# mingfeisun/DeepMimic_mujoco

Hardware: AMD Instinct MI355X
Metric: env-steps/sec (higher is better)
Workload: dtype f64

## Files before the change

### deepmimic_mujoco_amd/csrc/slot_step.h

```cpp
#pragma once

#include "env_step.h"
#include "slot_kernel.h"

namespace dm {

template <class R> struct DofVec { R r[DOF_PASSES]; };

template <class R>
DM_DEV void slot_integrate_pos(SlotShared<R>& s, const DofVec<R>& x0q, int sl, R h) {
  const R q0 = dmw::row_bcast<3>(x0q.r[0]), q1 = dmw::row_bcast<4>(x0q.r[0]), q2 = dmw::row_bcast<5>(x0q.r[0]), q3 = dmw::row_bcast<6>(x0q.r[0]);
  if (sl < 3) s.qpos[sl] = x0q.r[0] + h * s.tau[sl];
  else if (sl == 3) {
    R ax[3] = {s.tau[3], s.tau[4], s.tau[5]}, q[4] = {q0, q1, q2, q3}, qr[4];
    const R angle = h * normalize3(ax);
    if (angle == R(0)) { qr[0] = 1; qr[1] = qr[2] = qr[3] = 0; } else axisangle2quat(qr, ax, angle);
    normalize4(q);
    quat_mul(q, q, qr);
    s.qpos[3] = q[0]; s.qpos[4] = q[1]; s.qpos[5] = q[2]; s.qpos[6] = q[3];
  } else if (sl >= 7) s.qpos[sl] = x0q.r[0] + h * s.tau[sl - 1];
#pragma unroll
  for (int c = 1; c < Q_PASSES; c++) { const int i = sl + SW * c; if (i < NQ) s.qpos[i] = x0q.r[c] + h * s.tau[i - 1]; }
}

template <class R, bool PROF = false, bool CARRY = false, int MAXR = 2 * SW>
DM_DEV void slot_rk4_step(const DevModel<R>& M, SlotShared<R>& s, const SlotTables& tb, int sl, int lane, const LaneTopo& lt, R* xip, int& ovf, long long* prof = 0) {
  const R h = M.timestep;
  const R A[3] = {R(0.5), R(0.5), R(1)};
  const R Bw[4] = {R(1) / 6, R(1) / 3, R(1) / 3, R(1) / 6};
  DofVec<R> x0q, x0v, vprev, aprev, sumv, suma;
#pragma unroll
  for (int c = 0; c < DOF_PASSES; c++) {
    const int i = sl + SW * c;
    x0q.r[c] = i < NQ ? s.qpos[i] : R(0);
    const R v0 = i < NV ? s.qvel[i] : R(0);
    x0v.r[c] = v0; vprev.r[c] = v0; aprev.r[c] = 0; sumv.r[c] = 0; suma.r[c] = 0;
  }
  dmw::sync();
  for (int i = 0; i < 4; i++) {
    if (i > 0) {
      const R cf = A[i - 1];
#pragma unroll
      for (int c = 0; c < DOF_PASSES; c++) { const int d = sl + SW * c; if (d < NV) s.tau[d] = cf * vprev.r[c]; }
      dmw::sync();
      slot_integrate_pos(s, x0q, sl, h);
#pragma unroll
      for (int c = 0; c < DOF_PASSES; c++) {
        const int d = sl + SW * c;
        if (d < NV) { const R vi = x0v.r[c] + h * (cf * aprev.r[c]); vprev.r[c] = vi; s.qvel[d] = vi; }
      }
      dmw::sync();
    }
    typedef decltype(dmw::park(R(0))) ParkedR;
    ParkedR pk[5][DOF_PASSES];
#pragma unroll
    for (int c = 0; c < DOF_PASSES; c++) { pk[0][c] = dmw::park(x0q.r[c]); pk[1][c] = dmw::park(x0v.r[c]); pk[2][c] = dmw::park(vprev.r[c]); pk[3][c] = dmw::park(sumv.r[c]); pk[4][c] = dmw::park(suma.r[c]); }
    slot_forward<R, PROF, CARRY, MAXR>(M, s, tb, sl, lane, lt, xip, ovf, (const DebugOut*)0, prof);
#pragma unroll
    for (int c = 0; c < DOF_PASSES; c++) { x0q.r[c] = dmw::unpark(pk[0][c]); x0v.r[c] = dmw::unpark(pk[1][c]); vprev.r[c] = dmw::unpark(pk[2][c]); sumv.r[c] = dmw::unpark(pk[3][c]); suma.r[c] = dmw::unpark(pk[4][c]); }
#pragma unroll
    for (int c = 0; c < DOF_PASSES; c++) {
      const int d = sl + SW * c;
      if (d < NV) { const R a = s.qd.o.qacc[d]; aprev.r[c] = a; sumv.r[c] += Bw[i] * vprev.r[c]; suma.r[c] += Bw[i] * a; }
    }
  }
#pragma unroll
  for (int c = 0; c < DOF_PASSES; c++) { const int d = sl + SW * c; if (d < NV) s.tau[d] = sumv.r[c]; }
  dmw::sync();
  slot_integrate_pos(s, x0q, sl, h);
#pragma unroll
  for (int c = 0; c < DOF_PASSES; c++) { const int d = sl + SW * c; if (d < NV) { s.qvel[d] = x0v.r[c] + h * suma.r[c]; s.qws[d] = aprev.r[c]; } }
  dmw::sync();
}

template <class R>
DM_DEV void slot_load_env(const DevModel<R>& M, const Batch<R>& B, SlotShared<R>& s, int env, int sl, bool live, const double* action, int n_substeps = 1) {
#pragma unroll
  for (int c = 0; c < Q_PASSES; c++) {
    const int i = sl + SW * c;
    if (i < NQ) s.qpos[i] = B.qpos[(size_t)env * NQ + i];
    if (i < NV) { s.qvel[i] = B.qvel[(size_t)env * NV + i]; s.qws[i] = B.qws[(size_t)env * NV + i]; s.act[i] = 0; }
  }
  if (sl == 0) { s.status = 0; s.nefc = 0; s.ncon = 0; s.solver_iter = 0; }
  dmw::sync();
  if (action) {
#pragma unroll
    for (int c = 0; c < HINGE_PASSES; c++) {
      const int u = sl + SW * c;
      if (u < NU) {
        const R a = ctrl_of_action(M, B, env, u, (R)action[(size_t)env * NU + u], s.qpos[7 + u], s.qvel[6 + u], n_substeps);
        if (live) B.ctrl[(size_t)env * NU + u] = a;
        s.act[u + 6] = act_force(M, u + 6, a);
      }
    }
  }
  dmw::sync_mem();
}

template <class R, bool CARRY = false>
DM_DEV void slot_spd_control(const DevModel<R>& M, const Batch<R>& B, SlotShared<R>& s, const SlotTables& tb, int env, int sl, const LaneTopo& lt, bool live,
                             const DofVec<R>& qbar, const DofVec<R>& vbar) {
  const R h = M.timestep;
#pragma unroll
  for (int c = 0; c < DOF_PASSES; c++) { const int d = sl + SW * c; if (d < NV) s.act[d] = 0; }
  dmw::sync();
  R xip[3];
  bool skip_kin = false;
  if constexpr (CARRY) {
    skip_kin = dmw::ballot(s.kin_ok() != R(0)) == ~0ull;
    dmw::sync();
    if (sl == 0) s.kin_ok() = R(0);
  }
  if (!skip_kin) slot_kinematics(M, s, sl, lt, xip);
  slot_bias(M, s, tb, sl, lt);
  slot_mass_matrix<R, false, true>(M, s, tb, sl, lt, (const DebugOut*)0);
  R pd[DOF_PASSES], kd[DOF_PASSES];
#pragma unroll
  for (int c = 0; c < DOF_PASSES; c++) {
    const int d = sl + SW * c;
    pd[c] = 0; kd[c] = 0;
    if (d >= 6 && d < NV) {
      const R q = s.qpos[d + 1], v = s.qvel[d];
      kd[c] = M.kd[d];
      pd[c] = M.kp[d] * (qbar.r[c] - q - h * v) + kd[c] * (vbar.r[c] - v);
      s.tau[d] += pd[c];
    }
  }
  dmw::sync();
  {
    R x[1][NV];
#pragma unroll
    for (int d = 0; d < NV; d++) x[0][d] = s.tau[d];
    slot_solve_LT<1>(x, s.r2.qLD);
#pragma unroll
    for (int d = 0; d < NV; d++) { x[0][d] *= s.qd.o.dinv[d]; dmw::pin_value(x[0][d]); }
    solve_L(x[0], s.r2.qLD);
    if (sl == 0) {
#pragma unroll
      for (int d = 0; d < NV; d++) s.qd.o.qacc[d] = x[0][d];
    }
  }
  dmw::sync();
#pragma unroll
  for (int c = 0; c < DOF_PASSES; c++) {
    const int d = sl + SW * c;
    if (d >= 6 && d < NV) {
      const R ct = spd_ctrl(M, d, pd[c], kd[c], s.qd.o.qacc[d], h);
      if (live) B.ctrl[(size_t)env * NU + (d - 6)] = ct;
      s.act[d] = act_force(M, d, ct);
    }
  }
  dmw::sync_mem();
}

template <class R>
DM_DEV void slot_store_state(const Batch<R>& B, SlotShared<R>& s, int env, int sl, bool live) {
  if (!live) return;
#pragma unroll
  for (int c = 0; c < Q_PASSES; c++) {
    const int i = sl + SW * c;
    if (i < NQ) B.qpos[(size_t)env * NQ + i] = s.qpos[i];
    if (i < NV) { B.qvel[(size_t)env * NV + i] = s.qvel[i]; B.qws[(size_t)env * NV + i] = s.qws[i]; }
  }
}

template <class R>
DM_DEV void slot_reset_env(const DevModel<R>& M, const Batch<R>& B, SlotShared<R>& s, int env, int sl, bool doit, int mode, int hard) {
  const int ep = B.episode[env];
  const int genv = B.env_offset + env;
  const int idx = reset_draw(B, env, ep);
  if (doit) {
#pragma unroll
    for (int c = 0; c < Q_PASSES; c++) {
      const int i = sl + SW * c;
      if (i < NQ) {
        R q, v = 0;
        reset_element(M, B, mode, idx, genv, ep, i, q, v);
        s.qpos[i] = q;
        if (i < NV) s.qvel[i] = v;
      }
      if (hard && i < NV) s.qws[i] = 0;
    }
  }
  dmw::sync_mem();
  if (doit && sl == 0) reset_commit(B, env, ep, mode, hard, idx);
}
template <class R>
DM_DEV void slot_reset_env_clips(const DevModel<R>& M, const Batch<R>& B, const ClipArgs<R>& C, SlotShared<R>& s, int env, int sl, bool doit, int mode, int hard) {
  const int c = C.episode_clip(B, env, B.episode[env], mode, hard);
  slot_reset_env(M, clip_view(B, C.rec[c]), s, env, sl, doit, mode, hard);
  if (doit && sl == 0) C.clip[env] = c;
}

template <class R>
DM_DEV R slot_imitation_reward(const DevModel<R>& M, const Batch<R>& B, SlotShared<R>& s, int sl, const LaneTopo& lt, const R* ref, R shx, R shy, const R* refv = nullptr) {
  R qloc[4], aloc[3][3], xip[3];
  slot_kinematics(M, s, sl, lt, xip, qloc, aloc);
  const bool v1 = refv != nullptr;
  const R* rv = v1 ? refv : ref;
  const R* P = B.imit_pdev;
  R rq[4] = {s.qpos[3], s.qpos[4], s.qpos[5], s.qpos[6]};
  normalize4(rq);
  R pose = 0, vel = 0, eff = 0, root = 0, mx = 0, my = 0, mz = 0;
  if (sl < 13) {
    const int g = sl - 1;
    const int da = dmw::launder(lt.dofadr), nd = dmw::launder(lt.dofnum);
    const bool isroot = sl == 0, ball = !isroot && nd == 3;
    const R* rquat = ref + (isroot ? 3 : 13 + 4 * g);
    const R ident[4] = {1, 0, 0, 0};
    R q0[4], q1[4];
    for (int k = 0; k < 4; k++) { q0[k] = isroot ? rq[k] : (ball ? qloc[k] : ident[k]); q1[k] = (isroot || ball) ? rquat[k] : ident[k]; }
    const R th = quat_diff_theta(q0, q1);
    R pe = v1 ? fabs(th) : th * th, ve = 0;
    if (isroot) {
      R wv[3];
      const R wloc[3] = {s.qvel[3], s.qvel[4], s.qvel[5]};
      quat_rot(wv, rq, wloc);
      R dv2 = 0, dp2 = 0;
      for (int k = 0; k < 3; k++) { const R a = rv[10 + k] - wv[k]; ve += v1 ? fabs(a) : a * a; const R c = ref[7 + k] - s.qvel[k]; dv2 += c * c; }
      const R p1[3] = {ref[0] + shx, ref[1] + shy, ref[2]};
      for (int k = 0; k < 3; k++) { const R a = s.qpos[k] - p1[k]; dp2 += v1 ? fabs(a) : a * a; }
      root = v1 ? dp2 : dp2 + R(0.1) * pe + R(0.01) * dv2 + R(0.001) * ve;
    } else if (ball) {
      R wl[3] = {0, 0, 0};
      for (int k = 0; k < 3; k++) { const R rate = s.qvel[da + k]; wl[0] += aloc[k][0] * rate; wl[1] += aloc[k][1] * rate; wl[2] += aloc[k][2] * rate; }
      for (int k = 0; k < 3; k++) { const R w = rv[61 + 3 * g + k] - wl[k]; ve += v1 ? fabs(w) : w * w; }
    } else {
      const R a = ref[13 + 4 * g] - s.qpos[da + 1], w = rv[61 + 3 * g] - s.qvel[da];
      pe = v1 ? fabs(a) : a * a; ve = v1 ? fabs(w) + fabs(rv[61 + 3 * g + 1]) + fabs(rv[61 + 3 * g + 2]) : w * w;
    }
    const R wj = v1 ? (isroot ? R(1) : P[g] / P[12]) : P[isroot ? 12 : g];
    pose = wj * pe; vel = v1 ? ve : wj * ve;
  }
  if (sl < 4) {
    const int e = sl, b = (int)P[16 + e];
    const R ex[3] = {1, 0, 0};
    R fwd[3], p[3], rel[3];
    quat_rot(fwd, rq, ex);
    const R hn = sqrt(fwd[0] * fwd[0] + fwd[1] * fwd[1]);
    const R c = hn > R(0) ? fwd[0] / hn : R(1), sn = hn > R(0) ? fwd[1] / hn : R(0);
    mat_vec(p, s.xmat[b], P + 20 + 3 * e);
    for (int k = 0; k < 3; k++) { p[k] += s.xpos[b][k]; rel[k] = p[k] - s.qpos[k]; }
    rel[2] = p[2];
    const R f0[3] = {c * rel[0] + sn * rel[1], -sn * rel[0] + c * rel[1], rel[2]};
    for (int k = 0; k < 3; k++) { const R a = ref[97 + 3 * e + k] - f0[k]; eff += a * a; }
  }
#pragma unroll
  for (int cpass = 0; cpass < DOF_PASSES; cpass++) {
    const int d = sl + SW * cpass;
    if (d < NV) {
      const int b = TOPO.dof_body[d];
      const R* cb = s.r2.i.crb[b];
      const R* cd = s.cdof[d];
      const R qd = s.qvel[d], ms = cb[9];
      R axs[3];
      cross3(axs, cd, cb + 6);
      mx += qd * (ms * cd[3] + axs[0]); my += qd * (ms * cd[4] + axs[1]); mz += qd * (ms * cd[5] + axs[2]);
    }
  }
  pose = dmw::sum16(pose); vel = dmw::sum16(vel); eff = dmw::sum16(eff) / 4; root = dmw::row_bcast<0>(root);
  mx = dmw::sum16(mx) / M.total_mass; my = dmw::sum16(my) / M.total_mass; mz = dmw::sum16(mz) / M.total_mass;
  const R dc[3] = {ref[109] - mx, ref[110] - my, ref[111] - mz};
  const R com = R(0.1) * dot3(dc, dc);
  const R arg = sl == 0 ? R(-2) * pose : sl == 1 ? R(-0.1) * vel : sl == 2 ? (v1 ? R(-5) * root : R(-40) * eff) : sl == 3 ? R(-5) * root : R(-10) * com;
  const R wgt = sl == 0 ? R(0.5) : sl == 1 ? R(0.05) : sl == 2 ? (v1 ? R(0.2) : R(0.15)) : sl == 3 ? R(0.2) : R(0.1);
  R term = 0;
  if (sl < (v1 ? 3 : 5)) term = wgt * exp_once(arg);
  return dmw::sum16(term);
}

template <class R, bool PROF, bool CARRY, int MAXR, bool SPD, class CLIPS = NoClips>
DM_DEV bool slot_env_step_impl(const DevModel<R>& M, const Batch<R>& B, SlotShared<R>& s, SlotTables& tb, int env, int sl, int lane, bool live,
                               const double* action, double* obs, double* reward, unsigned char* done, int n_substeps, int* redo_count, int* redo_list,
                               long long* prof_out = 0, bool kin_carry = false, const CLIPS& clips = CLIPS()) {
  long long prof[32];
  for (int k = 0; k < 32; k++) prof[k] = 0;
  long long tstart = 0;
  if (PROF) tstart = dmw::clk();
  const LaneTopo lt = lane_topo(sl);
  if constexpr (CARRY) { if (!kin_carry && sl == 0) s.kin_ok() = R(0); }
  DofVec<R> qbar, vbar;
  {
  decltype(auto) Bv = clips.view(B, env);
  if constexpr (SPD) {
    slot_load_env(M, B, s, env, sl, live, (const double*)0);
#pragma unroll
    for (int c = 0; c < DOF_PASSES; c++) {
      const int d = sl + SW * c;
      qbar.r[c] = 0; vbar.r[c] = 0;
      if (d >= 6 && d < NV) spd_target(M, Bv, env, d - 6, action, n_substeps, qbar.r[c], vbar.r[c]);
    }
  } else
  slot_load_env(M, Bv, s, env, sl, live, action, n_substeps);
  }
  R xip[3];
  int why = 0;
  for (int k = 0; k < n_substeps; k++) {
    if constexpr (SPD) slot_spd_control<R, CARRY>(M, B, s, tb, env, sl, lt, live, qbar, vbar);
    slot_rk4_step<R, PROF, CARRY, MAXR>(M, s, tb, sl, lane, lt, xip, why, prof);
  }
  const bool ovf = dmw::row_ballot(why != 0, lane) != 0u;
  if (dmw::ballot(ovf) != 0ull) {
    unsigned bits = 0;
    for (int r = 0; r < 5; r++) if (dmw::row_ballot(((why >> r) & 1) != 0, lane) != 0u) bits |= 1u << r;
    if (ovf && live && sl == 0) {
      if (redo_count) { const int k = dmw::global_counter_next(redo_count); redo_list[k] = env; }
      for (int r = 0; r < 5; r++) if ((bits >> r) & 1u) dmw::global_counter_next(B.redo_why + 1 + r);
    }
  }
  live = live && !ovf;
  const R mz = sl < NB - 1 ? M.body_mass[sl + 1] * xip[2] : R(0);
  const R z = dmw::sum16(mz) / M.total_mass;
  bool dn = com_out_of_band(z);
  if (live) {
    if (B.diag != 0) {
      if (sl < NB - 1) for (int k = 0; k < 3; k++) B.xipos[(size_t)env * NB * 3 + 3 * (sl + 1) + k] = xip[k];
      if (sl < 3) B.xipos[(size_t)env * NB * 3 + sl] = 0;
      const int nc = s.ncon;
      for (int k = sl; k < MAXEFC * 2; k += SW) {
        const int c = k >> 1;
        int gid = -1;
        if (c < nc && c < SLOT_MAXCON) { const auto& rec = M.pair_rec[s.r1.rw.coni[c] & 0xff]; gid = (k & 1) ? rec.g2 : rec.g1; }
        B.cong[(size_t)env * MAXEFC * 2 + k] = gid;
      }
    }
    if (sl == 0) { B.comz[env] = z; B.ncon[env] = s.ncon; B.nefc[env] = s.nefc; B.status[env] = s.status; B.solver_iter[env] = s.solver_iter; if constexpr (!CARRY) order_ticket(B, env, s.nefc, s.solver_iter); }
  }
  R rew = 1;
  {
  decltype(auto) Bc = clips.view(B, env);
  if (B.reward_mode == REW_V3_CONFIG) {
    const FrameStep f = frame_step(REW_V3_CONFIG, M, Bc, n_substeps, B.frame_idx[env], 0, 0);
    R err = 0;
    for (int i = 7; i < NQ; i++) err += fabs(s.qpos[i] - Bc.mocap_cfg[(size_t)f.row * NQ + i]);
    rew = exp_once(-err);
    dmw::sync_mem();
    if (live && sl == 0) B.frame_idx[env] = f.store;
  } else if (B.reward_mode == REW_V2_POSE) {
    const FrameStep f = frame_step(REW_V2_POSE, M, Bc, n_substeps, B.frame_idx[env], B.frame_init[env], 0);
    R err = 0;
    for (int i = 3; i < NQ; i++) err += fabs(s.qpos[i] - Bc.mocap_cfg[(size_t)f.row * NQ + i]);
    const R acs = control_cost(B, env);
    rew = exp_once(R(-2) * err) - R(0.1) * acs;
    dmw::sync_mem();
    if (live && sl == 0) B.frame_idx[env] = f.store;
  } else if (B.reward_mode == REW_IMITATION) {
    const FrameStep f = frame_step(REW_IMITATION, M, Bc, n_substeps, B.frame_idx[env], 0, B.cycle[env]);
    rew = slot_imitation_reward(M, B, s, sl, lt, Bc.imit_table + (size_t)f.row * IMIT_FEAT, f.cycle * Bc.imit_params[13], f.cycle * Bc.imit_params[14]);
    dn = dn || f.ended;
    dmw::sync_mem();
    if (live && sl == 0) { B.frame_idx[env] = f.store; B.cycle[env] = f.cycle; }
  } else if (B.reward_mode == REW_V1_QUAT) {
    const FrameStep f = frame_step(REW_V1_QUAT, M, Bc, n_substeps, B.frame_idx[env], B.frame_init[env], 0);
    const R robs = slot_imitation_reward(M, B, s, sl, lt, Bc.imit_table + (size_t)f.row * IMIT_FEAT, R(0), R(0), Bc.imit_table + (size_t)f.row_v * IMIT_FEAT);
    const R acs = control_cost(B, env);
    rew = (f.take ? robs : R(0)) - R(0.1) * acs;
    dmw::sync_mem();
    if (live && sl == 0) B.frame_idx[env] = f.store;
  }
  }
  if (live && sl == 0) { B.time[env] += M.timestep * n_substeps; reward[env] = rew; done[env] = dn ? 1 : 0; if (B.kin) B.kin_ok[env] = 0; }
  if (B.autoreset) {
    dmw::sync_mem();
    if constexpr (CLIPS::on) slot_reset_env_clips(M, B, clips, s, env, sl, dn && live, B.autoreset == 1 ? 0 : 1, 1);
    else
    slot_reset_env(M, B, s, env, sl, dn && live, B.autoreset == 1 ? 0 : 1, 1);
  }
  if constexpr (CARRY) { if (sl == 0) s.kin_ok() = (B.reward_mode >= REW_IMITATION && !ovf && !(dn && B.autoreset != 0)) ? R(1) : R(0); }
  if (live) {
#pragma unroll
    for (int c = 0; c < (NOBS + SW - 1) / SW; c++) {
      const int o = sl + SW * c;
      if (o < NOBS) obs[(size_t)env * NOBS + o] = obs_element(s.qpos, s.qvel, o);
    }
  }
  slot_store_state(B, s, env, sl, live);
  if (PROF && lane == 0) {
    prof[5] = dmw::clk() - tstart;
    for (int k = 0; k < 32; k++) prof_out[k] = prof[k];
  }
  return live;
}
template <class R, bool PROF = false, bool CARRY = false, int MAXR = 2 * SW, class CLIPS = NoClips>
DM_DEV bool slot_env_step(const DevModel<R>& M, const Batch<R>& B, SlotShared<R>& s, SlotTables& tb, int env, int sl, int lane, bool live,
                          const double* action, double* obs, double* reward, unsigned char* done, int n_substeps, int* redo_count, int* redo_list,
                          long long* prof_out = 0, bool kin_carry = false, const CLIPS& clips = CLIPS()) {
  if (B.action_mode >= 3) return slot_env_step_impl<R, PROF, CARRY, MAXR, true, CLIPS>(M, B, s, tb, env, sl, lane, live, action, obs, reward, done, n_substeps, redo_count, redo_list, prof_out, kin_carry, clips);
  return slot_env_step_impl<R, PROF, CARRY, MAXR, false, CLIPS>(M, B, s, tb, env, sl, lane, live, action, obs, reward, done, n_substeps, redo_count, redo_list, prof_out, kin_carry, clips);
}

#ifdef DM_STATIC_CALLS
#define DM_CALL_SLOT_PARAM , int* call_slot
#define DM_CALL_SLOT_TOUCH(v) (*call_slot = (v))
#define DM_CALL_SLOT_ARG , &call_slot_mem
#define DM_CALL_SLOT_DECL int call_slot_mem = 0; asm volatile("" :: "v"(&call_slot_mem) : "memory")
#define DM_CALL_SLOT_USE asm volatile("" :: "v"(call_slot_mem))
#else
#define DM_CALL_SLOT_PARAM
#define DM_CALL_SLOT_TOUCH(v) ((void)0)
#define DM_CALL_SLOT_ARG
#define DM_CALL_SLOT_DECL ((void)0)
#define DM_CALL_SLOT_USE ((void)0)
#endif
template <class R> union SlotOrOne {
  SlotShared<R> sh[SLOTS];
  struct { Shared<R> s; StepScratch<R> x; } one;
};
template <class R, int NR, bool SPD = false>
DM_DEV_CALL64 void restep_one_env(const DevModel<R>* M, const Batch<R>* B, Shared<R>* s, StepScratch<R>* x, int env, int lane, const double* action, double* obs,
                                    double* reward, unsigned char* done, int n_substeps DM_CALL_SLOT_PARAM) {
  DM_CALL_SLOT_TOUCH(0);
  using dmw::uniform_ptr; using dmw::in_lds; using dmw::in_global; using dmw::in_constant;
  const Batch<R> Bv = *in_constant(B);
  env_step_impl<R, NR, false, SPD>(*in_constant(M), global_members(Bv), *in_lds(uniform_ptr(s)), *in_lds(uniform_ptr(x)), dmw::uniform(env), lane, in_global(uniform_ptr(action)),
                  in_global(uniform_ptr(obs)), in_global(uniform_ptr(reward)), in_global(uniform_ptr(done)), dmw::uniform(n_substeps));
}
template <class R, int MAXR, bool SPD = false>
DM_DEV_CALL64 int slot_env_step_call(const DevModel<R>* M, const Batch<R>* B, SlotShared<R>* s, SlotTables* tb, int env, int sl, int lane, bool live,
                                     const double* action, double* obs, double* reward, unsigned char* done, int n_substeps, int kin_carry DM_CALL_SLOT_PARAM) {
  using dmw::uniform_ptr; using dmw::in_lds; using dmw::in_global; using dmw::in_constant;
  const Batch<R> Bv = *in_constant(B);
  SlotShared<R>& sr = *in_lds(s);
  DM_CALL_SLOT_TOUCH(env);
  const bool stored = slot_env_step_impl<R, false, true, MAXR, SPD>(*in_constant(M), global_members(Bv), sr, *in_lds(uniform_ptr(tb)), env, sl, lane, live, in_global(uniform_ptr(action)),
                                                          in_global(uniform_ptr(obs)), in_global(uniform_ptr(reward)), in_global(uniform_ptr(done)), dmw::uniform(n_substeps), (int*)0, (int*)0,
                                                          (long long*)0, dmw::uniform(kin_carry) != 0);
  return (stored ? 1 : 0) | (sr.nefc << 8);
}
#ifdef DM_ROLLOUT_PROF
template <class R, int MAXR>
DM_DEV_CALL64 int slot_env_step_call_prof(const DevModel<R>* M, const Batch<R>* B, SlotShared<R>* s, SlotTables* tb, int env, int sl, int lane, bool live,
                                          const double* action, double* obs, double* reward, unsigned char* done, int n_substeps, long long* prof_out, int kin_carry DM_CALL_SLOT_PARAM) {
  DM_CALL_SLOT_TOUCH(env);
  using dmw::uniform_ptr; using dmw::in_lds; using dmw::in_global; using dmw::in_constant;
  const Batch<R> Bv = *in_constant(B);
  SlotShared<R>& sr = *in_lds(s);
  const bool stored = slot_env_step_impl<R, true, true, MAXR, false>(*in_constant(M), global_members(Bv), sr, *in_lds(uniform_ptr(tb)), env, sl, lane, live, in_global(uniform_ptr(action)),
                                                         in_global(uniform_ptr(obs)), in_global(uniform_ptr(reward)), in_global(uniform_ptr(done)), dmw::uniform(n_substeps), (int*)0, (int*)0,
                                                         in_global(uniform_ptr(prof_out)), dmw::uniform(kin_carry) != 0);
  return (stored ? 1 : 0) | (sr.nefc << 8);
}
#endif
struct StepRow { const double* action; double* obs; double* reward; unsigned char* done; };
#ifndef DM_EXT_MARGIN
#define DM_EXT_MARGIN 9
#endif
constexpr int EXT_MARGIN = DM_EXT_MARGIN;
struct NoTermination { static constexpr bool on = false; };
template <class T> struct TermSwitch { static constexpr bool on = T::on; };
template <class T> struct TermSwitch<T&> : TermSwitch<T> {};
template <class T> struct TermSwitch<const T> : TermSwitch<T> {};
template <class R, int NR, bool SPD = false, class POLICY, class TERM = NoTermination>
DM_DEV void slot_rollout(const DevModel<R>& M_in, const Batch<R>& B, SlotShared<R>* sh, SlotTables& tb, Shared<R>& one_s, StepScratch<R>& one_x,
                         int env, int lane, bool live, const StepRow* rows, int n_substeps, int T, POLICY&& policy, long long* prof_acc = 0, bool policy_clobbers_kin = false,
                         TERM&& term = TERM()) {
  const int slot = lane >> 4, sl = lane & 15;
  int carry = 0;
  int last_rows = B.nefc[env];
  DM_CALL_SLOT_DECL;
  for (int t = 0; t < T; t++) {
    const DevModel<R>& M = *dmw::launder_uniform_ptr(&M_in);
    const StepRow row = rows[t];
    const double* a_t = row.action;
    double* o_t = row.obs;
    double* r_t = row.reward;
    unsigned char* d_t = row.done;
    const bool heavy = rows_max(last_rows) > 2 * SW - EXT_MARGIN;
    int ret;
#ifdef DM_ROLLOUT_PROF
    if (prof_acc) {
      ret = heavy ? slot_env_step_call_prof<R, SLOT_MAXROWS>(&M, &B, &sh[slot], &tb, env, sl, lane, live, a_t, o_t, r_t, d_t, n_substeps, prof_acc + 32, carry DM_CALL_SLOT_ARG)
                  : slot_env_step_call_prof<R, 2 * SW>(&M, &B, &sh[slot], &tb, env, sl, lane, live, a_t, o_t, r_t, d_t, n_substeps, prof_acc + 32, carry DM_CALL_SLOT_ARG);
      if (lane == 0) { for (int k = 0; k < 31; k++) prof_acc[k] += prof_acc[32 + k]; if (heavy) prof_acc[28] += 1; }
    } else
#endif
    ret = heavy ? slot_env_step_call<R, SLOT_MAXROWS, SPD>(&M, &B, &sh[slot], &tb, env, sl, lane, live, a_t, o_t, r_t, d_t, n_substeps, carry DM_CALL_SLOT_ARG)
                : slot_env_step_call<R, 2 * SW, SPD>(&M, &B, &sh[slot], &tb, env, sl, lane, live, a_t, o_t, r_t, d_t, n_substeps, carry DM_CALL_SLOT_ARG);
    const bool stored = (ret & 1) != 0;
    last_rows = (stored || !live) ? (ret >> 8) : SLOT_MAXROWS;
    const int need = (live && !stored) ? 1 : 0;
    bool any = false;
    for (int k = 0; k < SLOTS; k++) {
      if (dmw::bcast_i(need, SW * k) == 0) continue;
      any = true;
      const int e = dmw::bcast_i(env, SW * k);
      dmw::sync_mem();
      restep_one_env<R, NR, SPD>(&M, &B, &one_s, &one_x, e, lane, a_t, o_t, r_t, d_t, n_substeps DM_CALL_SLOT_ARG);
      if (lane == 0) dmw::global_counter_next(B.redo_why);
      dmw::sync_mem();
    }
    if constexpr (TermSwitch<TERM>::on) term(&M, &B, &sh[slot], t, env, sl, lane, live, any, o_t, d_t DM_CALL_SLOT_ARG);
    if (any) {
#pragma unroll
      for (int c = 0; c < (NOBS + SW - 1) / SW; c++) {
        const int o = sl + SW * c;
        if (o < 28) sh[slot].qpos[7 + o] = (R)o_t[(size_t)env * NOBS + o];
        else if (o < NOBS) sh[slot].qvel[6 + (o - 28)] = (R)o_t[(size_t)env * NOBS + o];
      }
      dmw::sync_mem();
    }
    DM_CALL_SLOT_USE;
    policy(t);
    carry = (any || policy_clobbers_kin) ? 0 : 1;
    dmw::sync_mem();
  }
}

}
```

### deepmimic_mujoco_amd/csrc/step_rules.h

```cpp
#pragma once

#include "dmenv.h"
#include "env_kernel.h"

namespace dm {

template <class R>
struct Batch {
  R* qpos;
  R* qvel;
  R* qws;
  R* time;
  R* ctrl;
  R* xipos;
  R* comz;
  int* frame_idx;
  int* frame_init;
  int* ncon;
  int* nefc;
  int* cong;
  R* aovf;
  int* status;
  int* solver_iter;
  int* episode;
  int* order;
  const int* ord_in;
  const int* ordl_in;
  int* ord_out;
  int* ordl_out;
  int* ord_zero;
  int ord_stride;
  int* cycle;
  R* kin;
  unsigned char* kin_ok;
  int* redo_list;
  int* redo_count;
  int* redo_why;
  const R* mocap_cfg;
  const R* mocap_vel;
  const R* imit_table;
  const R* imit_pdev;
  R imit_params[32];
  R mocap_dt;
  int n_frames;
  int n_envs;
  int env_offset;
  int reward_mode, autoreset, action_mode;
  int diag;
  unsigned long long seed;
};

template <class R>
DM_DEV Batch<R> global_members(Batch<R> b) {
  using dmw::in_global;
  b.qpos = in_global(b.qpos); b.qvel = in_global(b.qvel); b.qws = in_global(b.qws); b.time = in_global(b.time); b.ctrl = in_global(b.ctrl);
  b.xipos = in_global(b.xipos); b.comz = in_global(b.comz); b.frame_idx = in_global(b.frame_idx); b.frame_init = in_global(b.frame_init);
  b.ncon = in_global(b.ncon); b.nefc = in_global(b.nefc); b.cong = in_global(b.cong); b.aovf = in_global(b.aovf); b.status = in_global(b.status);
  b.solver_iter = in_global(b.solver_iter); b.episode = in_global(b.episode); b.order = in_global(b.order); b.cycle = in_global(b.cycle);
  b.kin = in_global(b.kin); b.kin_ok = in_global(b.kin_ok); b.redo_list = in_global(b.redo_list); b.redo_count = in_global(b.redo_count);
  b.redo_why = in_global(b.redo_why); b.mocap_cfg = in_global(b.mocap_cfg); b.mocap_vel = in_global(b.mocap_vel);
  b.imit_table = in_global(b.imit_table); b.imit_pdev = in_global(b.imit_pdev);
  return b;
}

DM_DEV unsigned long long mix64(unsigned long long z) {
  z += 0x9E3779B97F4A7C15ull;
  z = (z ^ (z >> 30)) * 0xBF58476D1CE4E5B9ull;
  z = (z ^ (z >> 27)) * 0x94D049BB133111EBull;
  return z ^ (z >> 31);
}
DM_DEV double rng_uniform(unsigned long long seed, int genv, int episode, int k) {
  unsigned long long h = mix64(seed ^ mix64((unsigned long long)(unsigned)genv * 0x100000001B3ull + 0x1234567ull));
  h = mix64(h ^ ((unsigned long long)(unsigned)episode << 32 | (unsigned)k));
  return (double)(h >> 11) * (1.0 / 9007199254740992.0);
}

template <class R>
struct ClipRec { int row0, n_frames; R dt, loop, shift_x, shift_y; double cdf; };
template <class R>
DM_DEV Batch<R> clip_view(Batch<R> b, const ClipRec<R>& r) {
  b.mocap_cfg += (size_t)r.row0 * NQ; b.mocap_vel += (size_t)r.row0 * NV;
  if (b.imit_table) b.imit_table += (size_t)r.row0 * IMIT_FEAT;
  b.n_frames = r.n_frames; b.mocap_dt = r.dt;
  b.imit_params[13] = r.shift_x; b.imit_params[14] = r.shift_y; b.imit_params[15] = r.loop;
  return b;
}
struct NoClips {
  static constexpr bool on = false;
  template <class R> DM_DEV const Batch<R>& view(const Batch<R>& B, int) const { return B; }
  template <class R> DM_DEV const Batch<R>& view_uniform(const Batch<R>& B, int) const { return B; }
};
template <class R>
struct ClipArgs {
  static constexpr bool on = true;
  int* clip;
  const ClipRec<R>* rec;
  int n_clips, mode;
  DM_DEV Batch<R> view(const Batch<R>& B, int env) const { return clip_view(B, rec[clip[env]]); }
  DM_DEV Batch<R> view_uniform(const Batch<R>& B, int env) const { return clip_view(B, rec[dmw::uniform(clip[env])]); }
  DM_DEV int episode_clip(const Batch<R>& B, int env, int ep, int reset_mode, int hard) const {
    if (mode != 1 || !(reset_mode == 0 || (reset_mode == 1 && hard))) return clip[env];
    const double u = rng_uniform(B.seed, B.env_offset + env, ep, 128);
    int c = 0;
    while (c < n_clips - 1 && !(u < rec[c].cdf)) c++;
    return c;
  }
};

template <class R>
DM_DEV int v1_update_interval(const DevModel<R>& M, const Batch<R>& B, int n_substeps) {
  int upd = (int)floor(B.mocap_dt / (M.timestep * n_substeps));
  if (upd < 1) upd = 1;
  return upd;
}

template <class R>
DM_DEV int step_start_frame(const DevModel<R>& M, const Batch<R>& B, int env, int n_substeps) {
  const int idx = B.frame_idx[env];
  if (B.reward_mode == REW_V2_POSE) return (idx + B.frame_init[env]) % B.n_frames;
  if (B.reward_mode == REW_V1_QUAT) return (idx / v1_update_interval(M, B, n_substeps) + B.frame_init[env]) % B.n_frames;
  return idx;
}

template <class R>
DM_DEV void set_frame(const Batch<R>& B, int env, int idx) {
  B.frame_init[env] = idx;
  B.frame_idx[env] = (B.reward_mode == REW_V2_POSE || B.reward_mode == REW_V1_QUAT) ? 0 : idx;
  B.cycle[env] = 0;
}

struct FrameStep { int store, row, row_v, cycle; bool ended, take; };
template <class R>
DM_DEV FrameStep frame_step(int mode, const DevModel<R>& M, const Batch<R>& B, int n_substeps, int idx, int init, int cyc) {
  FrameStep f = {idx + 1, idx, idx, cyc, false, true};
  if (mode == REW_V3_CONFIG) f.store = (idx + 1) % B.n_frames;
  else if (mode == REW_V2_POSE) f.row = (f.store + init) % B.n_frames;
  else if (mode == REW_IMITATION) {
    if (f.store >= B.n_frames) { if (B.imit_params[15] != R(0)) { f.store = 0; f.cycle += 1; } else { f.store = B.n_frames - 1; f.ended = true; } }
    f.row = f.store;
  } else if (mode == REW_V1_QUAT) {
    const int upd = v1_update_interval(M, B, n_substeps);
    f.take = f.store % upd == 0;
    f.row = (f.store / upd + init) % B.n_frames;
    f.row_v = f.row + 1 < B.n_frames ? f.row + 1 : B.n_frames - 1;
  }
  return f;
}

template <class R>
DM_DEV R ctrl_of_action(const DevModel<R>& M, const Batch<R>& B, int env, int u, R a, R q_u, R v_u, int n_substeps) {
  if (B.action_mode == 1) {
    const int idx = step_start_frame(M, B, env, n_substeps);
    a += R(0.8) * (B.mocap_cfg[(size_t)idx * NQ + 7 + u] - q_u);
  } else if (B.action_mode == 2) {
    const int idx = step_start_frame(M, B, env, n_substeps);
    a += M.kp[u + 6] * (B.mocap_cfg[(size_t)idx * NQ + 7 + u] - q_u) + M.kd[u + 6] * (B.mocap_vel[(size_t)idx * NV + 6 + u] - v_u);
  }
  return a;
}
template <class R>
DM_DEV void spd_target(const DevModel<R>& M, const Batch<R>& B, int env, int u, const double* action, int n_substeps, R& qbar, R& vbar) {
  qbar = 0; vbar = 0;
  if (action) qbar = (R)action[(size_t)env * NU + u];
  if (B.action_mode == 4) {
    const int idx = step_start_frame(M, B, env, n_substeps);
    qbar += B.mocap_cfg[(size_t)idx * NQ + 7 + u];
    vbar = B.mocap_vel[(size_t)idx * NV + 6 + u];
  }
}
template <class R>
DM_DEV R spd_ctrl(const DevModel<R>& M, int d, R p_plus_d, R kd, R qacc, R h) { return (p_plus_d - h * kd * qacc) / M.gear[d]; }
template <class R>
DM_DEV R act_force(const DevModel<R>& M, int d, R ctrl) { return M.gear[d] * clampr(ctrl, M.ctrl_lo[d], M.ctrl_hi[d]); }

template <class R>
DM_DEV R control_cost(const Batch<R>& B, int env) {
  R acs = 0;
  for (int u = 0; u < NU; u++) { const R c = B.ctrl[(size_t)env * NU + u]; acs += c * c; }
  return acs;
}
template <class R>
DM_DEV bool com_out_of_band(R z) { return (z < R(0.7)) || (z > R(2.0)); }

template <class R>
DM_DEV R obs_element(const R* qpos, const R* qvel, int o) { return o < 28 ? qpos[7 + o] : qvel[6 + (o - 28)]; }

template <class R>
DM_DEV int reset_draw(const Batch<R>& B, int env, int ep) {
  const int idx = (int)(rng_uniform(B.seed, B.env_offset + env, ep, 0) * (double)B.n_frames);
  return idx >= B.n_frames ? B.n_frames - 1 : idx;
}
template <class R>
DM_DEV void reset_element(const DevModel<R>& M, const Batch<R>& B, int mode, int idx, int genv, int ep, int i, R& q, R& v) {
  if (mode == 0) {
    q = B.mocap_cfg[(size_t)idx * NQ + i];
    if (i < NV) v = B.mocap_vel[(size_t)idx * NV + i];
  } else if (mode == 1) {
    q = M.qpos0[i] + (R)((rng_uniform(B.seed, genv, ep, 1 + i) * 2.0 - 1.0) * 0.01);
    if (i < NV) v = (R)((rng_uniform(B.seed, genv, ep, 64 + i) * 2.0 - 1.0) * 0.01);
  } else {
    q = M.qpos0[i];
    v = 0;
  }
}
template <class R>
DM_DEV void reset_commit(const Batch<R>& B, int env, int ep, int mode, int hard, int idx) {
  if (hard) B.time[env] = 0;
  B.episode[env] = ep + 1;
  if (mode == 0 || (mode == 1 && hard)) set_frame(B, env, idx); else B.cycle[env] = 0;
}

struct TermVerdict {
  bool stepdone, limit;
  int steps;
  DM_DEV bool ends(bool fall) const { return !stepdone && (fall || limit); }
  DM_DEV int reason(bool fall) const { return stepdone ? DM_DONE_STEP : ((fall ? DM_DONE_FALL : 0) | (limit ? DM_DONE_TIME_LIMIT : 0)); }
  DM_DEV int steps_kept(bool fall) const { return (stepdone || fall || limit) ? 0 : steps; }
};
DM_DEV TermVerdict term_verdict(bool stepdone, int steps_before, int max_steps) {
  const int steps = steps_before + 1;
  return TermVerdict{stepdone, max_steps > 0 && steps >= max_steps, steps};
}
template <class R>
DM_DEV int trunc_index_value(int j, int env, int tick, const Batch<R>& B) { return j == 0 ? env : (j == 1 ? tick : (j == 2 ? B.frame_idx[env] : B.frame_init[env])); }

}
```

Before: 20.97 million.

## Hoist global loads ahead of syncs and skip resets when no lane resets

Global reads in env load, reset, reward and termination paths (state, actions, gear/limits, mocap rows, reference features, frame indices, time) are issued into registers up front behind a scheduling fence, so their latency overlaps with other work. It also returns early from reset when no lane in the wavefront needs it, merges the post-reward stores into one block with a single sync_mem, and threads a time load through the reward via a callback. This is meant to hide global-memory latency in the per-step epilogue and prologue, at the cost of more registers and unconditional loads of data that may go unused.

```diff
diff --git a/deepmimic_mujoco_amd/csrc/slot_step.h b/deepmimic_mujoco_amd/csrc/slot_step.h
--- a/deepmimic_mujoco_amd/csrc/slot_step.h
+++ b/deepmimic_mujoco_amd/csrc/slot_step.h
@@ -75,22 +75,57 @@
 
 template <class R>
 DM_DEV void slot_load_env(const DevModel<R>& M, const Batch<R>& B, SlotShared<R>& s, int env, int sl, bool live, const double* action, int n_substeps = 1) {
+  R q_in[Q_PASSES], v_in[Q_PASSES], w_in[Q_PASSES];
+#pragma unroll
+  for (int c = 0; c < Q_PASSES; c++) {
+    const int i = sl + SW * c, iq = i < NQ ? i : 0, iv = i < NV ? i : 0;
+    q_in[c] = B.qpos[(size_t)env * NQ + iq]; v_in[c] = B.qvel[(size_t)env * NV + iv]; w_in[c] = B.qws[(size_t)env * NV + iv];
+  }
+  const bool tracks = action && (B.action_mode == 1 || B.action_mode == 2);
+  R a_in[HINGE_PASSES] = {}, gear[HINGE_PASSES] = {}, lo[HINGE_PASSES] = {}, hi[HINGE_PASSES] = {};
+  int cur = 0, init = 0;
+  if (action) {
+#pragma unroll
+    for (int c = 0; c < HINGE_PASSES; c++) {
+      const int u = sl + SW * c, uu = u < NU ? u : 0;
+      a_in[c] = (R)action[(size_t)env * NU + uu];
+      gear[c] = M.gear[uu + 6]; lo[c] = M.ctrl_lo[uu + 6]; hi[c] = M.ctrl_hi[uu + 6];
+    }
+    if (tracks) {
+      cur = B.frame_idx[env];
+      if (B.reward_mode == REW_V2_POSE || B.reward_mode == REW_V1_QUAT) init = B.frame_init[env];
+    }
+  }
+  dmw::sched_fence();
 #pragma unroll
   for (int c = 0; c < Q_PASSES; c++) {
     const int i = sl + SW * c;
-    if (i < NQ) s.qpos[i] = B.qpos[(size_t)env * NQ + i];
-    if (i < NV) { s.qvel[i] = B.qvel[(size_t)env * NV + i]; s.qws[i] = B.qws[(size_t)env * NV + i]; s.act[i] = 0; }
+    if (i < NQ) s.qpos[i] = q_in[c];
+    if (i < NV) { s.qvel[i] = v_in[c]; s.qws[i] = w_in[c]; s.act[i] = 0; }
   }
   if (sl == 0) { s.status = 0; s.nefc = 0; s.ncon = 0; s.solver_iter = 0; }
   dmw::sync();
   if (action) {
+    R cfg[HINGE_PASSES], vel[HINGE_PASSES], kp[HINGE_PASSES], kd[HINGE_PASSES];
+#pragma unroll
+    for (int c = 0; c < HINGE_PASSES; c++) { cfg[c] = 0; vel[c] = 0; kp[c] = 0; kd[c] = 0; }
+    if (tracks) {
+      const int idx = step_start_frame(M, B, n_substeps, cur, init);
+#pragma unroll
+      for (int c = 0; c < HINGE_PASSES; c++) {
+        const int u = sl + SW * c, uu = u < NU ? u : 0;
+        cfg[c] = B.mocap_cfg[(size_t)idx * NQ + 7 + uu];
+        if (B.action_mode == 2) { vel[c] = B.mocap_vel[(size_t)idx * NV + 6 + uu]; kp[c] = M.kp[uu + 6]; kd[c] = M.kd[uu + 6]; }
+      }
+      dmw::sched_fence();
+    }
 #pragma unroll
     for (int c = 0; c < HINGE_PASSES; c++) {
       const int u = sl + SW * c;
       if (u < NU) {
-        const R a = ctrl_of_action(M, B, env, u, (R)action[(size_t)env * NU + u], s.qpos[7 + u], s.qvel[6 + u], n_substeps);
+        const R a = ctrl_of_action(B, a_in[c], s.qpos[7 + u], s.qvel[6 + u], cfg[c], vel[c], kp[c], kd[c]);
         if (live) B.ctrl[(size_t)env * NU + u] = a;
-        s.act[u + 6] = act_force(M, u + 6, a);
+        s.act[u + 6] = act_force(gear[c], lo[c], hi[c], a);
       }
     }
   }
@@ -166,15 +201,27 @@
 
 template <class R>
 DM_DEV void slot_reset_env(const DevModel<R>& M, const Batch<R>& B, SlotShared<R>& s, int env, int sl, bool doit, int mode, int hard) {
+  if (dmw::ballot(doit) == 0ull) return;
   const int ep = B.episode[env];
   const int genv = B.env_offset + env;
   const int idx = reset_draw(B, env, ep);
+  R q_in[Q_PASSES] = {}, v_in[Q_PASSES] = {};
+  if (mode == 0) {
+#pragma unroll
+    for (int c = 0; c < Q_PASSES; c++) {
+      const int i = sl + SW * c, iq = i < NQ ? i : 0, iv = i < NV ? i : 0;
+      q_in[c] = B.mocap_cfg[(size_t)idx * NQ + iq]; v_in[c] = B.mocap_vel[(size_t)idx * NV + iv];
+    }
+    dmw::sched_fence();
+  }
   if (doit) {
 #pragma unroll
     for (int c = 0; c < Q_PASSES; c++) {
       const int i = sl + SW * c;
       if (i < NQ) {
         R q, v = 0;
+        if (mode == 0) reset_element_rsi(i, q_in[c], v_in[c], q, v);
+        else
         reset_element(M, B, mode, idx, genv, ep, i, q, v);
         s.qpos[i] = q;
         if (i < NV) s.qvel[i] = v;
@@ -187,29 +234,42 @@
 }
 template <class R>
 DM_DEV void slot_reset_env_clips(const DevModel<R>& M, const Batch<R>& B, const ClipArgs<R>& C, SlotShared<R>& s, int env, int sl, bool doit, int mode, int hard) {
+  if (dmw::ballot(doit) == 0ull) return;
   const int c = C.episode_clip(B, env, B.episode[env], mode, hard);
   slot_reset_env(M, clip_view(B, C.rec[c]), s, env, sl, doit, mode, hard);
   if (doit && sl == 0) C.clip[env] = c;
 }
 
-template <class R>
-DM_DEV R slot_imitation_reward(const DevModel<R>& M, const Batch<R>& B, SlotShared<R>& s, int sl, const LaneTopo& lt, const R* ref, R shx, R shy, const R* refv = nullptr) {
+struct NoRide { DM_DEV void operator()() const {} };
+template <class R, class RIDE = NoRide>
+DM_DEV R slot_imitation_reward(const DevModel<R>& M, const Batch<R>& B, SlotShared<R>& s, int sl, const LaneTopo& lt, const R* ref, R shx, R shy, const R* refv = nullptr,
+                               const RIDE& ride = RIDE()) {
   R qloc[4], aloc[3][3], xip[3];
   slot_kinematics(M, s, sl, lt, xip, qloc, aloc);
   const bool v1 = refv != nullptr;
   const R* rv = v1 ? refv : ref;
   const R* P = B.imit_pdev;
+  const int gl = sl >= 1 && sl < 13 ? sl - 1 : 0, el = sl < 4 ? sl : 0;
+  const int qoff = sl == 0 || sl >= 13 ? 3 : 13 + 4 * gl, roff = sl == 0 || sl >= 13 ? 10 : 61 + 3 * gl;
+  R ref_q[4], ref_w[3], ref_p[3], ref_v[3], ref_e[3], ref_c[3], p_off[3];
+  for (int k = 0; k < 4; k++) ref_q[k] = ref[qoff + k];
+  for (int k = 0; k < 3; k++) { ref_w[k] = rv[roff + k]; ref_p[k] = ref[k]; ref_v[k] = ref[7 + k]; ref_e[k] = ref[97 + 3 * el + k]; ref_c[k] = ref[109 + k]; p_off[k] = P[20 + 3 * el + k]; }
+  const R p_w = P[sl == 0 || sl >= 13 ? 12 : gl], p_12 = P[12], p_body = P[16 + el];
+  const R total_mass = M.total_mass;
+  int dof_b[DOF_PASSES];
+#pragma unroll
+  for (int cpass = 0; cpass < DOF_PASSES; cpass++) { const int d = sl + SW * cpass; dof_b[cpass] = TOPO.dof_body[d < NV ? d : 0]; }
+  ride();
+  dmw::sched_fence();
   R rq[4] = {s.qpos[3], s.qpos[4], s.qpos[5], s.qpos[6]};
   normalize4(rq);
   R pose = 0, vel = 0, eff = 0, root = 0, mx = 0, my = 0, mz = 0;
   if (sl < 13) {
-    const int g = sl - 1;
     const int da = dmw::launder(lt.dofadr), nd = dmw::launder(lt.dofnum);
     const bool isroot = sl == 0, ball = !isroot && nd == 3;
-    const R* rquat = ref + (isroot ? 3 : 13 + 4 * g);
     const R ident[4] = {1, 0, 0, 0};
     R q0[4], q1[4];
-    for (int k = 0; k < 4; k++) { q0[k] = isroot ? rq[k] : (ball ? qloc[k] : ident[k]); q1[k] = (isroot || ball) ? rquat[k] : ident[k]; }
+    for (int k = 0; k < 4; k++) { q0[k] = isroot ? rq[k] : (ball ? qloc[k] : ident[k]); q1[k] = (isroot || ball) ? ref_q[k] : ident[k]; }
     const R th = quat_diff_theta(q0, q1);
     R pe = v1 ? fabs(th) : th * th, ve = 0;
     if (isroot) {
@@ -217,39 +277,39 @@
       const R wloc[3] = {s.qvel[3], s.qvel[4], s.qvel[5]};
       quat_rot(wv, rq, wloc);
       R dv2 = 0, dp2 = 0;
-      for (int k = 0; k < 3; k++) { const R a = rv[10 + k] - wv[k]; ve += v1 ? fabs(a) : a * a; const R c = ref[7 + k] - s.qvel[k]; dv2 += c * c; }
-      const R p1[3] = {ref[0] + shx, ref[1] + shy, ref[2]};
+      for (int k = 0; k < 3; k++) { const R a = ref_w[k] - wv[k]; ve += v1 ? fabs(a) : a * a; const R c = ref_v[k] - s.qvel[k]; dv2 += c * c; }
+      const R p1[3] = {ref_p[0] + shx, ref_p[1] + shy, ref_p[2]};
       for (int k = 0; k < 3; k++) { const R a = s.qpos[k] - p1[k]; dp2 += v1 ? fabs(a) : a * a; }
       root = v1 ? dp2 : dp2 + R(0.1) * pe + R(0.01) * dv2 + R(0.001) * ve;
     } else if (ball) {
       R wl[3] = {0, 0, 0};
       for (int k = 0; k < 3; k++) { const R rate = s.qvel[da + k]; wl[0] += aloc[k][0] * rate; wl[1] += aloc[k][1] * rate; wl[2] += aloc[k][2] * rate; }
-      for (int k = 0; k < 3; k++) { const R w = rv[61 + 3 * g + k] - wl[k]; ve += v1 ? fabs(w) : w * w; }
+      for (int k = 0; k < 3; k++) { const R w = ref_w[k] - wl[k]; ve += v1 ? fabs(w) : w * w; }
     } else {
-      const R a = ref[13 + 4 * g] - s.qpos[da + 1], w = rv[61 + 3 * g] - s.qvel[da];
-      pe = v1 ? fabs(a) : a * a; ve = v1 ? fabs(w) + fabs(rv[61 + 3 * g + 1]) + fabs(rv[61 + 3 * g + 2]) : w * w;
-    }
-    const R wj = v1 ? (isroot ? R(1) : P[g] / P[12]) : P[isroot ? 12 : g];
+      const R a = ref_q[0] - s.qpos[da + 1], w = ref_w[0] - s.qvel[da];
+      pe = v1 ? fabs(a) : a * a; ve = v1 ? fabs(w) + fabs(ref_w[1]) + fabs(ref_w[2]) : w * w;
+    }
+    const R wj = v1 ? (isroot ? R(1) : p_w / p_12) : p_w;
     pose = wj * pe; vel = v1 ? ve : wj * ve;
   }
   if (sl < 4) {
-    const int e = sl, b = (int)P[16 + e];
+    const int b = (int)p_body;
     const R ex[3] = {1, 0, 0};
     R fwd[3], p[3], rel[3];
     quat_rot(fwd, rq, ex);
     const R hn = sqrt(fwd[0] * fwd[0] + fwd[1] * fwd[1]);
     const R c = hn > R(0) ? fwd[0] / hn : R(1), sn = hn > R(0) ? fwd[1] / hn : R(0);
-    mat_vec(p, s.xmat[b], P + 20 + 3 * e);
+    mat_vec(p, s.xmat[b], p_off);
     for (int k = 0; k < 3; k++) { p[k] += s.xpos[b][k]; rel[k] = p[k] - s.qpos[k]; }
     rel[2] = p[2];
     const R f0[3] = {c * rel[0] + sn * rel[1], -sn * rel[0] + c * rel[1], rel[2]};
-    for (int k = 0; k < 3; k++) { const R a = ref[97 + 3 * e + k] - f0[k]; eff += a * a; }
+    for (int k = 0; k < 3; k++) { const R a = ref_e[k] - f0[k]; eff += a * a; }
   }
 #pragma unroll
   for (int cpass = 0; cpass < DOF_PASSES; cpass++) {
     const int d = sl + SW * cpass;
     if (d < NV) {
-      const int b = TOPO.dof_body[d];
+      const int b = dof_b[cpass];
       const R* cb = s.r2.i.crb[b];
       const R* cd = s.cdof[d];
       const R qd = s.qvel[d], ms = cb[9];
@@ -259,8 +319,8 @@
     }
   }
   pose = dmw::sum16(pose); vel = dmw::sum16(vel); eff = dmw::sum16(eff) / 4; root = dmw::row_bcast<0>(root);
-  mx = dmw::sum16(mx) / M.total_mass; my = dmw::sum16(my) / M.total_mass; mz = dmw::sum16(mz) / M.total_mass;
-  const R dc[3] = {ref[109] - mx, ref[110] - my, ref[111] - mz};
+  mx = dmw::sum16(mx) / total_mass; my = dmw::sum16(my) / total_mass; mz = dmw::sum16(mz) / total_mass;
+  const R dc[3] = {ref_c[0] - mx, ref_c[1] - my, ref_c[2] - mz};
   const R com = R(0.1) * dot3(dc, dc);
   const R arg = sl == 0 ? R(-2) * pose : sl == 1 ? R(-0.1) * vel : sl == 2 ? (v1 ? R(-5) * root : R(-40) * eff) : sl == 3 ? R(-5) * root : R(-10) * com;
   const R wgt = sl == 0 ? R(0.5) : sl == 1 ? R(0.05) : sl == 2 ? (v1 ? R(0.2) : R(0.15)) : sl == 3 ? R(0.2) : R(0.1);
@@ -309,72 +369,79 @@
     }
   }
   live = live && !ovf;
-  const R mz = sl < NB - 1 ? M.body_mass[sl + 1] * xip[2] : R(0);
+  const int ev = dmw::launder(env);
+  const int rmode = B.reward_mode;
+  const R body_mass = M.body_mass[sl < NB - 1 ? sl + 1 : 1];
+  const int cur = B.frame_idx[ev], cur_init = B.frame_init[ev], cur_cycle = B.cycle[ev];
+  R tval = 0;
+  if (rmode < REW_IMITATION) tval = B.time[ev];
+  dmw::sched_fence();
+  const R mz = sl < NB - 1 ? body_mass * xip[2] : R(0);
   const R z = dmw::sum16(mz) / M.total_mass;
   bool dn = com_out_of_band(z);
   if (live) {
     if (B.diag != 0) {
-      if (sl < NB - 1) for (int k = 0; k < 3; k++) B.xipos[(size_t)env * NB * 3 + 3 * (sl + 1) + k] = xip[k];
-      if (sl < 3) B.xipos[(size_t)env * NB * 3 + sl] = 0;
+      if (sl < NB - 1) for (int k = 0; k < 3; k++) B.xipos[(size_t)ev * NB * 3 + 3 * (sl + 1) + k] = xip[k];
+      if (sl < 3) B.xipos[(size_t)ev * NB * 3 + sl] = 0;
       const int nc = s.ncon;
       for (int k = sl; k < MAXEFC * 2; k += SW) {
         const int c = k >> 1;
         int gid = -1;
         if (c < nc && c < SLOT_MAXCON) { const auto& rec = M.pair_rec[s.r1.rw.coni[c] & 0xff]; gid = (k & 1) ? rec.g2 : rec.g1; }
-        B.cong[(size_t)env * MAXEFC * 2 + k] = gid;
+        B.cong[(size_t)ev * MAXEFC * 2 + k] = gid;
       }
     }
-    if (sl == 0) { B.comz[env] = z; B.ncon[env] = s.ncon; B.nefc[env] = s.nefc; B.status[env] = s.status; B.solver_iter[env] = s.solver_iter; if constexpr (!CARRY) order_ticket(B, env, s.nefc, s.solver_iter); }
   }
   R rew = 1;
+  FrameStep f = {0, 0, 0, 0, false, true};
   {
-  decltype(auto) Bc = clips.view(B, env);
-  if (B.reward_mode == REW_V3_CONFIG) {
-    const FrameStep f = frame_step(REW_V3_CONFIG, M, Bc, n_substeps, B.frame_idx[env], 0, 0);
+  decltype(auto) Bc = clips.view(B, ev);
+  const auto clock_rides = [&]() { tval = B.time[ev]; };
+  if (rmode == REW_V3_CONFIG) {
+    f = frame_step(REW_V3_CONFIG, M, Bc, n_substeps, cur, 0, 0);
     R err = 0;
     for (int i = 7; i < NQ; i++) err += fabs(s.qpos[i] - Bc.mocap_cfg[(size_t)f.row * NQ + i]);
     rew = exp_once(-err);
-    dmw::sync_mem();
-    if (live && sl == 0) B.frame_idx[env] = f.store;
-  } else if (B.reward_mode == REW_V2_POSE) {
-    const FrameStep f = frame_step(REW_V2_POSE, M, Bc, n_substeps, B.frame_idx[env], B.frame_init[env], 0);
+  } else if (rmode == REW_V2_POSE) {
+    f = frame_step(REW_V2_POSE, M, Bc, n_substeps, cur, cur_init, 0);
     R err = 0;
     for (int i = 3; i < NQ; i++) err += fabs(s.qpos[i] - Bc.mocap_cfg[(size_t)f.row * NQ + i]);
-    const R acs = control_cost(B, env);
+    const R acs = control_cost(B, ev);
     rew = exp_once(R(-2) * err) - R(0.1) * acs;
-    dmw::sync_mem();
-    if (live && sl == 0) B.frame_idx[env] = f.store;
-  } else if (B.reward_mode == REW_IMITATION) {
-    const FrameStep f = frame_step(REW_IMITATION, M, Bc, n_substeps, B.frame_idx[env], 0, B.cycle[env]);
-    rew = slot_imitation_reward(M, B, s, sl, lt, Bc.imit_table + (size_t)f.row * IMIT_FEAT, f.cycle * Bc.imit_params[13], f.cycle * Bc.imit_params[14]);
+  } else if (rmode == REW_IMITATION) {
+    f = frame_step(REW_IMITATION, M, Bc, n_substeps, cur, 0, cur_cycle);
+    rew = slot_imitation_reward(M, B, s, sl, lt, Bc.imit_table + (size_t)f.row * IMIT_FEAT, f.cycle * Bc.imit_params[13], f.cycle * Bc.imit_params[14], (const R*)nullptr, clock_rides);
     dn = dn || f.ended;
-    dmw::sync_mem();
-    if (live && sl == 0) { B.frame_idx[env] = f.store; B.cycle[env] = f.cycle; }
-  } else if (B.reward_mode == REW_V1_QUAT) {
-    const FrameStep f = frame_step(REW_V1_QUAT, M, Bc, n_substeps, B.frame_idx[env], B.frame_init[env], 0);
-    const R robs = slot_imitation_reward(M, B, s, sl, lt, Bc.imit_table + (size_t)f.row * IMIT_FEAT, R(0), R(0), Bc.imit_table + (size_t)f.row_v * IMIT_FEAT);
-    const R acs = control_cost(B, env);
+  } else if (rmode == REW_V1_QUAT) {
+    f = frame_step(REW_V1_QUAT, M, Bc, n_substeps, cur, cur_init, 0);
+    const R robs = slot_imitation_reward(M, B, s, sl, lt, Bc.imit_table + (size_t)f.row * IMIT_FEAT, R(0), R(0), Bc.imit_table + (size_t)f.row_v * IMIT_FEAT, clock_rides);
+    const R acs = control_cost(B, ev);
     rew = (f.take ? robs : R(0)) - R(0.1) * acs;
-    dmw::sync_mem();
-    if (live && sl == 0) B.frame_idx[env] = f.store;
-  }
-  }
-  if (live && sl == 0) { B.time[env] += M.timestep * n_substeps; reward[env] = rew; done[env] = dn ? 1 : 0; if (B.kin) B.kin_ok[env] = 0; }
+  }
+  }
+  dmw::sync_mem();
+  if (live && sl == 0) {
+    B.comz[ev] = z; B.ncon[ev] = s.ncon; B.nefc[ev] = s.nefc; B.status[ev] = s.status; B.solver_iter[ev] = s.solver_iter;
+    if constexpr (!CARRY) order_ticket(B, ev, s.nefc, s.solver_iter);
+    if (rmode != 0) B.frame_idx[ev] = f.store;
+    if (rmode == REW_IMITATION) B.cycle[ev] = f.cycle;
+    tval += M.timestep * n_substeps;
+    B.time[ev] = tval; reward[ev] = rew; done[ev] = dn ? 1 : 0; if (B.kin) B.kin_ok[ev] = 0;
+  }
   if (B.autoreset) {
-    dmw::sync_mem();
-    if constexpr (CLIPS::on) slot_reset_env_clips(M, B, clips, s, env, sl, dn && live, B.autoreset == 1 ? 0 : 1, 1);
+    if constexpr (CLIPS::on) slot_reset_env_clips(M, B, clips, s, ev, sl, dn && live, B.autoreset == 1 ? 0 : 1, 1);
     else
-    slot_reset_env(M, B, s, env, sl, dn && live, B.autoreset == 1 ? 0 : 1, 1);
+    slot_reset_env(M, B, s, ev, sl, dn && live, B.autoreset == 1 ? 0 : 1, 1);
   }
   if constexpr (CARRY) { if (sl == 0) s.kin_ok() = (B.reward_mode >= REW_IMITATION && !ovf && !(dn && B.autoreset != 0)) ? R(1) : R(0); }
   if (live) {
 #pragma unroll
     for (int c = 0; c < (NOBS + SW - 1) / SW; c++) {
       const int o = sl + SW * c;
-      if (o < NOBS) obs[(size_t)env * NOBS + o] = obs_element(s.qpos, s.qvel, o);
-    }
-  }
-  slot_store_state(B, s, env, sl, live);
+      if (o < NOBS) obs[(size_t)ev * NOBS + o] = obs_element(s.qpos, s.qvel, o);
+    }
+  }
+  slot_store_state(B, s, ev, sl, live);
   if (PROF && lane == 0) {
     prof[5] = dmw::clk() - tstart;
     for (int k = 0; k < 32; k++) prof_out[k] = prof[k];
diff --git a/deepmimic_mujoco_amd/csrc/step_rules.h b/deepmimic_mujoco_amd/csrc/step_rules.h
--- a/deepmimic_mujoco_amd/csrc/step_rules.h
+++ b/deepmimic_mujoco_amd/csrc/step_rules.h
@@ -115,11 +115,16 @@
 }
 
 template <class R>
+DM_DEV int step_start_frame(const DevModel<R>& M, const Batch<R>& B, int n_substeps, int idx, int init) {
+  if (B.reward_mode == REW_V2_POSE) return (idx + init) % B.n_frames;
+  if (B.reward_mode == REW_V1_QUAT) return (idx / v1_update_interval(M, B, n_substeps) + init) % B.n_frames;
+  return idx;
+}
+template <class R>
 DM_DEV int step_start_frame(const DevModel<R>& M, const Batch<R>& B, int env, int n_substeps) {
   const int idx = B.frame_idx[env];
-  if (B.reward_mode == REW_V2_POSE) return (idx + B.frame_init[env]) % B.n_frames;
-  if (B.reward_mode == REW_V1_QUAT) return (idx / v1_update_interval(M, B, n_substeps) + B.frame_init[env]) % B.n_frames;
-  return idx;
+  const bool two = B.reward_mode == REW_V2_POSE || B.reward_mode == REW_V1_QUAT;
+  return step_start_frame(M, B, n_substeps, idx, two ? B.frame_init[env] : 0);
 }
 
 template <class R>
@@ -148,15 +153,20 @@
 }
 
 template <class R>
+DM_DEV R ctrl_of_action(const Batch<R>& B, R a, R q_u, R v_u, R cfg, R vel, R kp, R kd) {
+  if (B.action_mode == 1) a += R(0.8) * (cfg - q_u);
+  else if (B.action_mode == 2) a += kp * (cfg - q_u) + kd * (vel - v_u);
+  return a;
+}
+template <class R>
 DM_DEV R ctrl_of_action(const DevModel<R>& M, const Batch<R>& B, int env, int u, R a, R q_u, R v_u, int n_substeps) {
-  if (B.action_mode == 1) {
+  R cfg = 0, vel = 0, kp = 0, kd = 0;
+  if (B.action_mode == 1 || B.action_mode == 2) {
     const int idx = step_start_frame(M, B, env, n_substeps);
-    a += R(0.8) * (B.mocap_cfg[(size_t)idx * NQ + 7 + u] - q_u);
-  } else if (B.action_mode == 2) {
-    const int idx = step_start_frame(M, B, env, n_substeps);
-    a += M.kp[u + 6] * (B.mocap_cfg[(size_t)idx * NQ + 7 + u] - q_u) + M.kd[u + 6] * (B.mocap_vel[(size_t)idx * NV + 6 + u] - v_u);
-  }
-  return a;
+    cfg = B.mocap_cfg[(size_t)idx * NQ + 7 + u];
+    if (B.action_mode == 2) { vel = B.mocap_vel[(size_t)idx * NV + 6 + u]; kp = M.kp[u + 6]; kd = M.kd[u + 6]; }
+  }
+  return ctrl_of_action(B, a, q_u, v_u, cfg, vel, kp, kd);
 }
 template <class R>
 DM_DEV void spd_target(const DevModel<R>& M, const Batch<R>& B, int env, int u, const double* action, int n_substeps, R& qbar, R& vbar) {
@@ -171,7 +181,9 @@
 template <class R>
 DM_DEV R spd_ctrl(const DevModel<R>& M, int d, R p_plus_d, R kd, R qacc, R h) { return (p_plus_d - h * kd * qacc) / M.gear[d]; }
 template <class R>
-DM_DEV R act_force(const DevModel<R>& M, int d, R ctrl) { return M.gear[d] * clampr(ctrl, M.ctrl_lo[d], M.ctrl_hi[d]); }
+DM_DEV R act_force(R gear, R lo, R hi, R ctrl) { return gear * clampr(ctrl, lo, hi); }
+template <class R>
+DM_DEV R act_force(const DevModel<R>& M, int d, R ctrl) { return act_force(M.gear[d], M.ctrl_lo[d], M.ctrl_hi[d], ctrl); }
 
 template <class R>
 DM_DEV R control_cost(const Batch<R>& B, int env) {
@@ -191,10 +203,13 @@
   return idx >= B.n_frames ? B.n_frames - 1 : idx;
 }
 template <class R>
+DM_DEV void reset_element_rsi(int i, R cfg, R vel, R& q, R& v) { q = cfg; if (i < NV) v = vel; }
+template <class R>
 DM_DEV void reset_element(const DevModel<R>& M, const Batch<R>& B, int mode, int idx, int genv, int ep, int i, R& q, R& v) {
   if (mode == 0) {
-    q = B.mocap_cfg[(size_t)idx * NQ + i];
-    if (i < NV) v = B.mocap_vel[(size_t)idx * NV + i];
+    R vel = 0;
+    if (i < NV) vel = B.mocap_vel[(size_t)idx * NV + i];
+    reset_element_rsi(i, B.mocap_cfg[(size_t)idx * NQ + i], vel, q, v);
   } else if (mode == 1) {
     q = M.qpos0[i] + (R)((rng_uniform(B.seed, genv, ep, 1 + i) * 2.0 - 1.0) * 0.01);
     if (i < NV) v = (R)((rng_uniform(B.seed, genv, ep, 64 + i) * 2.0 - 1.0) * 0.01);
```

Measured after the change: 21.19 million, median of 6. 1.1% higher.
